# nightgoodl/ovmono3d

Measured on AMD Instinct MI355X. Metric: images/sec/GPU @512x512 DINOv2-L SFP; AP3D delta vs reference, higher is better.
Workload: dtype f16x3; 1 GPU; DINOv2 vitl14 + SFP + ROIHeads3DGDINO (native GroundingDINO Swin-B/BERT-base, 900 queries, 6 categories -> NMS) + ROIAlign + CubeHead + decode, batch 1/GPU, 512x512 synthetic -> network res 532 -> canvas 896 (T=4097), random-init weights (seed 0); precision=f16x3, parallelism=dp1 (image-sharded, no data-path collective)

## Files before the change

### ovmono3d_amd/csrc/gdino.hip

```cpp
#include <cmath>
#include <cstdio>
#include <cstdlib>
#include "det2d.hpp"
#include "dec_chain.hpp"
#include "gdino_model.hpp"

using namespace ovm;
using namespace ovm::gdino;

namespace ovm {
GdinoTune g_gdino_tune = {1, 1, 0, 1, 1, 1, 0};
void set_gdino_branches(int v) { g_gdino_tune.branches = v ? 1 : 0; }
void set_gdino_dec_chain(int v) { g_gdino_tune.dec_chain = v ? 1 : 0; }
void set_gdino_ffn_split(int v) { g_gdino_tune.ffn_split = v ? 1 : 0; }
void set_gdino_swin_fused(int v) { g_gdino_tune.swin_fused = v ? 1 : 0; }
void set_gdino_swin_tap(int v) { g_gdino_tune.swin_tap = v > 0 ? v : 0; }
void set_gdino_gemm256(int v) { g_gdino_tune.gemm256 = v ? 1 : 0; }
void set_gdino_mlp_fused(int v) { g_gdino_tune.mlp_fused = v < 0 ? 0 : (v > 2 ? 2 : v); }
}

namespace ovm {
namespace gdino {
namespace {

struct Feat { float* f; int h, w, C; };
struct DecScratch {
  float *tkv_all, *val_all;
  float *sine, *qh, *qpos, *qk, *vq, *ctx, *pre, *ow, *ffb, *b1, *b2, *delta;
  float* refs[2];
  bool chain; int ffn_chunks;
  float *ffn_x, *ffn_part;
};
struct State {
  float *tx, *text0, *text;
  std::vector<Feat> feats;
  float *vis0, *vis;
  float* ref; int* topk;
  float *hs, *last_ref, *hn;
  DecScratch d;
};

inline int now_cols(const OvmGdinoConfig& c) { return c.heads * c.n_levels * c.n_points * 3; }

void mha_core(Run& r, const float* q, int ldq, const float* k, int ldk, const float* v, int ldv, int Tq, int Tk, int heads, int D, const float* bias,
              int ldb, float* out, int ldo) {
  AttnF32Params a; memset(&a, 0, sizeof(a));
  const int dh = D / heads;
  a.q = q; a.k = k; a.v = v; a.ldq = ldq; a.ldk = ldk; a.ldv = ldv;
  a.sq2 = dh; a.sk2 = dh; a.sv2 = dh; a.o = out; a.ldo = ldo; a.so2 = dh;
  a.nb1 = 1; a.nb2 = heads; a.Tq = Tq; a.Tk = Tk; a.DH = dh; a.scale = 1.0f / sqrtf((float)dh);
  a.bias_b = bias; a.sbb = 0; a.ldbb = ldb;
// ... 129 lines not shown
    r.rowop(p);
    float* y = r.f32((size_t)h * w * C);
    GemmParams q = r.gp(pa, h * w, g->pe); q.C = y; q.ldc = C;
    r.gemm(q, EPI_STORE);
    r.ln(y, h * w, C, g->pe_ln, eps, nullptr, x);
    r.release(mk);
  }
  int ordinal = 0;
  for (size_t si = 0; si < g->stages.size(); ++si) {
    const SwinStage& stg = g->stages[si];
    const StageGeo& ge = pl->geo[si];
    const int ntok = h * w;
    for (size_t b = 0; b < stg.blocks.size(); ++b) swin_block(r, stg.blocks[b], ge.wm[b & 1], x, C, stg.nh, ntok, ++ordinal);
    if (stg.has_out) {
      float* f = r.f32((size_t)ntok * C);
      r.ln(x, ntok, C, stg.on, eps, nullptr, f);
      st.feats.push_back({f, h, w, C});
      r.tap("swin_stage" + std::to_string(st.feats.size()), f, (int64_t)ntok * C);
    }
    if (stg.has_red) { x = patch_merge(r, stg, ge, x, C); h = ge.h2; w = ge.w2; C = 2 * C; }
  }
}

void neck(Run& r, State& st) {
  OvmGdino* g = r.g; Plan* pl = r.pl;
  const OvmGdinoConfig& c = g->cfg;
  const int D = c.d_model, S = pl->S;
  st.vis0 = r.f32((size_t)S * D);
  st.vis = r.f32((size_t)S * D);
  const size_t mk = r.mark();
  for (int l = 0; l < c.n_levels; ++l) {
    const int n = pl->lh[l] * pl->lw[l];
    float* y = r.f32((size_t)n * D);
    const bool conv = l >= (int)st.feats.size();
    const Feat& f = conv ? st.feats.back() : st.feats[l];
    const int K = conv ? 9 * f.C : f.C;
    SplitBuf a = r.split((size_t)n, K);
    RowOpParams p = Run::rows(f.f, f.C, n, K); Run::into(p, a);
    if (conv) { p.idx = pl->conv_map; p.nidx = 9; p.seg = f.C; }
    r.rowop(p);
    GemmParams q = r.gp(a, n, g->inproj[l].w); q.C = y; q.ldc = D;
    r.gemm(q, EPI_STORE);
    if (r.go()) r.chk(ovm_g_groupnorm(y, 1, n, D, 32, g->inproj[l].gn.g, g->inproj[l].gn.b, 1e-5f, st.vis0 + (size_t)pl->lstart[l] * D, r.s_main), "groupnorm");
  }
  r.release(mk);
}

struct EncBufs {
  float* v; SplitBuf vsp; float *t, *qvv, *tkv; SplitBuf cv; float* ct;
  BiAttnWs bw; float *sc, *stat, *part, *bml;
  float *text2, *tqk, *tv, *tctx, *tff;
  SplitBuf vis_sp, visp_sp; float *val, *ow; SplitBuf dsp; float* pre; SplitBuf ff;
  bool ffn_fused;
};

void fusion_layer(Run& r, const EncLayer& ly, EncBufs& b, const float* vis_in, const float* text_in) {
  const OvmGdinoConfig& c = r.g->cfg;
  const int D = c.d_model, T = r.pl->T, S = r.pl->S, HF = c.heads / 2, E = c.ffn_dim / 2, dhf = E / HF;
  r.ln(vis_in, S, D, ly.lnv, c.eps, nullptr, b.v, &b.vsp);
  r.ln(text_in, T, D, ly.lnt, c.eps, nullptr, b.t);
  { GemmParams q = r.gp(b.vsp, S, ly.vqv); q.C = b.qvv; q.ldc = 2 * E; r.gemm(q, EPI_STORE); }
  r.lin(b.t, nullptr, D, T, ly.tkv, 0, nullptr, 0, b.tkv, 2 * E);
  if (!r.go()) return;
  BiAttnParams a; memset(&a, 0, sizeof(a));
  a.qv = b.qvv; a.ldq = 2 * E; a.kt = b.tkv; a.ldk = 2 * E; a.vv = b.qvv + E; a.ldvv = 2 * E; a.vt = b.tkv + E; a.ldvt = 2 * E;
  a.S = S; a.T = T; a.H = HF; a.dh = dhf; a.scale = 1.0f / sqrtf((float)dhf);
  a.cv_hi = b.cv.hi; a.cv_lo = b.cv.lo; a.ldcv = b.cv.ld; a.ct = b.ct; a.sc = b.sc; a.stat = b.stat; a.part = b.part; a.chunk = b.bw.chunk; a.nchunk = b.bw.nchunk;
// ... 5 lines not shown
  const OvmGdinoConfig& c = r.g->cfg;
  const int D = c.d_model, T = r.pl->T, E = c.ffn_dim / 2;
  r.fork(); r.on_text();
  r.lin(b.ct, nullptr, E, T, ly.ot, 0, b.t, D, b.text2, D);
  r.lin(b.text2, r.pl->text_pos, D, T, ly.te.qk, 0, nullptr, 0, b.tqk, 2 * D);
  r.lin(b.text2, nullptr, D, T, ly.te.v, 0, nullptr, 0, b.tv, D);
  mha_core(r, b.tqk, 2 * D, b.tqk + D, 2 * D, b.tv, D, T, T, ly.te.heads, D, r.pl->text_bias, T, b.tctx, D);
  r.lin(b.tctx, nullptr, D, T, ly.te.out, 0, b.text2, D, b.t, D);
  r.ln(b.t, T, D, ly.te_ln1, c.eps, nullptr, b.text2);
  r.lin(b.text2, nullptr, D, T, ly.te_fc1, 1, nullptr, 0, b.tff, ly.te_fc1.N);
  r.lin(b.tff, nullptr, ly.te_fc1.N, T, ly.te_fc2, 0, b.text2, D, b.t, D);
  r.ln(b.t, T, D, ly.te_ln2, c.eps, nullptr, text);
  r.on_image();
}

void deformable_layer(Run& r, const EncLayer& ly, EncBufs& b, float* vis) {
  const OvmGdinoConfig& c = r.g->cfg; Plan* pl = r.pl;
  const int D = c.d_model, S = pl->S, NOW = now_cols(c);
  { GemmParams q = r.gp(b.cv, S, ly.ov); q.C = vis; q.ldc = D; q.R = b.v; q.ldr = D; r.gemm(q, EPI_STORE); }
  {
    RowOpParams p = Run::rows(vis, D, S, D); Run::into(p, b.vis_sp);
    p.add = pl->pos; p.ld_add = D; p.add_rows = S; p.hi2 = b.visp_sp.hi; p.lo2 = b.visp_sp.lo; p.ldh2 = b.visp_sp.ld;
    r.rowop(p);
  }
  { GemmParams q = r.gp(b.vis_sp, S, ly.msda.value); q.C = b.val; q.ldc = D; r.gemm(q, EPI_STORE); }
  { GemmParams q = r.gp(b.visp_sp, S, ly.msda.offw); q.C = b.ow; q.ldc = NOW; r.gemm(q, EPI_STORE); }
  deform(r, b.val, D, b.ow, NOW, pl->ref, 2, 0, S, nullptr, &b.dsp);
  { GemmParams q = r.gp(b.dsp, S, ly.msda.out); q.C = b.pre; q.ldc = D; q.R = vis; q.ldr = D; r.gemm(q, EPI_STORE); }
  r.ln(b.pre, S, D, ly.de_ln1, c.eps, nullptr, b.v, &b.vsp);
  if (b.ffn_fused) {
    GemmParams q = r.gp(b.vsp, S, ly.de_fc2); q.C = b.pre; q.ldc = D; q.R = b.v; q.ldr = D;
    r.mlp_fused(b.vsp, S, ly.de_fc1, ly.de_fc2, 1, q, EPI_STORE);
  } else {
    { GemmParams q = r.gp(b.vsp, S, ly.de_fc1); q.Ohi = b.ff.hi; q.Olo = b.ff.lo; q.ldo = b.ff.ld; q.relu = 1; r.gemm(q, EPI_STORE); }
    { GemmParams q = r.gp(b.ff, S, ly.de_fc2); q.C = b.pre; q.ldc = D; q.R = b.v; q.ldr = D; r.gemm(q, EPI_STORE); }
  }
  r.ln(b.pre, S, D, ly.de_ln2, c.eps, nullptr, vis);
}

void encoder(Run& r, State& st) {
  const OvmGdinoConfig& c = r.g->cfg;
  const int D = c.d_model, T = r.pl->T, S = r.pl->S, HF = c.heads / 2, E = c.ffn_dim / 2, dhf = E / HF;
  r.join();
  const size_t mk = r.mark();
  EncBufs b;
  b.v = r.f32((size_t)S * D); b.vsp = r.split_for256((size_t)S, D);
  b.t = r.f32((size_t)T * D);
  b.qvv = r.f32((size_t)S * 2 * E);
  b.tkv = r.f32((size_t)T * 2 * E);
  b.cv = r.split((size_t)S, E);
  b.ct = r.f32((size_t)T * E);
  b.bw = biattn_workspace(S, T, HF, dhf, false);
  b.sc = b.bw.sc ? r.f32(b.bw.sc) : nullptr;
  b.stat = b.bw.stat ? r.f32(b.bw.stat) : nullptr;
  b.part = r.f32(b.bw.part);
  b.bml = b.bw.ml ? r.f32(2 * b.bw.ml) : nullptr;
  b.text2 = r.f32((size_t)T * D);
  b.tqk = r.f32((size_t)T * 2 * D); b.tv = r.f32((size_t)T * D); b.tctx = r.f32((size_t)T * D);
  b.tff = r.f32((size_t)T * c.ffn_dim);
  b.vis_sp = r.split((size_t)S, D); b.visp_sp = r.split((size_t)S, D);
  b.val = r.f32((size_t)S * D);
  b.ow = r.f32((size_t)S * now_cols(c));
  b.dsp = r.split((size_t)S, D);
  b.pre = r.f32((size_t)S * D);
  b.ffn_fused = b.vsp.il;
  for (auto& ly : r.g->enc) b.ffn_fused = b.ffn_fused && r.mlp_fused_ok(2, S, ly.de_fc1, ly.de_fc2, 1);
  if (!b.ffn_fused) b.ff = r.split((size_t)S, c.ffn_dim);
  const float* vis_in = st.vis0; const float* text_in = st.text0;
  for (auto& ly : r.g->enc) {
    fusion_layer(r, ly, b, vis_in, text_in);
    vis_in = st.vis; text_in = st.text;
    text_enhancer(r, ly, b, st.text);
    deformable_layer(r, ly, b, st.vis);
    r.join();
  }
  r.release(mk);
  r.tap("source_flatten", st.vis0, (int64_t)S * D);
  r.tap("enc_vision", st.vis, (int64_t)S * D);
  r.tap("enc_text", st.text, (int64_t)T * D);
}

void select_queries(Run& r, State& st) {
  OvmGdino* g = r.g; Plan* pl = r.pl;
  const OvmGdinoConfig& c = g->cfg;
  const int D = c.d_model, T = pl->T, S = pl->S, Q = c.num_queries;
  const hipStream_t s = r.s_main;
  float* ref = st.ref = r.f32((size_t)Q * 4);
  int* topk = st.topk = r.i32((size_t)Q);
// ... 26 lines not shown
  r.tap("topk", topk, Q);
  r.tap("init_ref", ref, (int64_t)Q * 4);
}

size_t decoder_inputs(Run& r, State& st) {
  OvmGdino* g = r.g; Plan* pl = r.pl;
  const OvmGdinoConfig& c = g->cfg;
  const int D = c.d_model, T = pl->T, S = pl->S, Q = c.num_queries, NL = (int)g->dec.size();
  DecScratch& d = st.d;
  st.hs = r.f32((size_t)Q * D);
  st.last_ref = r.f32((size_t)Q * 4);
  st.hn = r.f32((size_t)Q * D);
  const size_t mk = r.mark();
  d.tkv_all = r.f32((size_t)T * NL * 2 * D);
  r.lin(st.text, nullptr, D, T, g->dec_kv_text, 0, nullptr, 0, d.tkv_all, NL * 2 * D);
  SplitBuf vsp = r.split_for256((size_t)S, D);
  { RowOpParams p = Run::rows(st.vis, D, S, D); Run::into(p, vsp); r.rowop(p); }
  d.val_all = r.f32((size_t)S * NL * D);
  { GemmParams q = r.gp(vsp, S, g->dec_value); q.C = d.val_all; q.ldc = NL * D; r.gemm(q, EPI_STORE); }
  r.copy(st.hs, g->tgt, sizeof(float) * (size_t)Q * D, r.s_main);
  d.sine = r.f32((size_t)Q * 2 * D);
  d.qh = r.f32((size_t)Q * D); d.qpos = r.f32((size_t)Q * D);
  d.qk = r.f32((size_t)Q * 2 * D); d.vq = r.f32((size_t)Q * D); d.ctx = r.f32((size_t)Q * D);
  d.pre = r.f32((size_t)Q * D);
  d.ow = r.f32((size_t)Q * now_cols(c));
  d.ffb = r.f32((size_t)Q * c.ffn_dim);
  d.b1 = r.f32((size_t)Q * D); d.b2 = r.f32((size_t)Q * D); d.delta = r.f32((size_t)Q * 4);
  d.refs[0] = st.ref; d.refs[1] = r.f32((size_t)Q * 4);
  d.chain = pl->tune.dec_chain && dec_chain_supported(D, c.heads, c.ffn_dim, c.n_levels, c.n_points, T, g->precision);
  const int chunks = c.ffn_dim > 512 ? c.ffn_dim / 512 : 1;
  d.ffn_chunks = (d.chain && pl->tune.ffn_split && chunks > 1) ? chunks : 0;
  d.ffn_x = d.ffn_chunks ? r.f32((size_t)Q * D) : nullptr;
// ... 173 lines not shown
    (void)hipDeviceGetStreamPriorityRange(&lo, &hi);
    if (hipStreamCreateWithPriority(&g->aux, hipStreamNonBlocking, hi) != hipSuccess || hipEventCreateWithFlags(&g->ev_fork, hipEventDisableTiming) != hipSuccess ||
        hipEventCreateWithFlags(&g->ev_join, hipEventDisableTiming) != hipSuccess) {
      g->err = "could not create the text-branch stream"; return OVM_ERR_HIP;
    }
  }
  const OvmGdinoConfig& c = g->cfg;
  if (c.d_model % c.heads || c.n_levels > 8 || c.n_levels < 1 || c.swin_window <= 0) { g->err = "bad GroundingDINO config"; return OVM_ERR_INVALID; }
  OVM_HIP(g, hipSetDevice(device));
  const WeightMap wm(weights, n_weights);
  OVM_TRY(g, load_bert(g, wm));
  OVM_TRY(g, load_swin(g, wm));
  OVM_TRY(g, load_neck(g, wm));
  OVM_TRY(g, load_encoder(g, wm));
  OVM_TRY(g, load_decoder(g, wm));
  OVM_HIP(g, hipDeviceSynchronize());
  return OVM_OK;
}

int ovm_gdino_destroy(OvmGdino* g) {
  if (!g) return OVM_OK;
  (void)hipSetDevice(g->device);
  (void)hipDeviceSynchronize();
  for (Plan* p : g->plans) delete p;
  g->free_all();
  if (g->aux) (void)hipStreamDestroy(g->aux);
  if (g->ev_fork) (void)hipEventDestroy(g->ev_fork);
  if (g->ev_join) (void)hipEventDestroy(g->ev_join);
  delete g;
  return OVM_OK;
// ... 85 lines not shown
```

### ovmono3d_amd/csrc/gdino_load.hip

```cpp
#include <cmath>
#include "gdino_model.hpp"

namespace ovm {
namespace gdino {
namespace {

const std::string M = "model.";

int up_ln(OvmGdino* g, const WeightMap& wm, const std::string& prefix, Ln* ln) {
  OVM_TRY(g, upload_weight(g, wm, prefix + ".weight", -1, &ln->g));
  return upload_weight(g, wm, prefix + ".bias", -1, &ln->b);
}

int make_frag(OvmGdino* g, Lin* w) {
  std::vector<half_t> src; src.swap(w->img);
  if (g->precision != 3 || !w->hi) return OVM_OK;
  const int Npad = npad128(w->N), KS = w->Kpad / 32;
  const size_t n = (size_t)Npad * 2 * w->Kpad;
  if (src.size() != n) { g->err = "make_frag: the weight was packed without keeping its host image"; return OVM_ERR_INVALID; }
  std::vector<half_t> dst(n);
  for (int tile = 0; tile < Npad / 16; ++tile)
    for (int ks = 0; ks < KS; ++ks)
      for (int part = 0; part < 2; ++part)
        for (int lane = 0; lane < 64; ++lane) {
// ... 196 lines not shown
  {
    const int F = c.d_model / 2;
    std::vector<float> dt((size_t)F / 2);
    for (int i = 0; i < F / 2; ++i) dt[i] = powf(10000.0f, 2.f * (float)i / (float)F);
    OVM_TRY(g, upload_f32(g, dt.data(), dt.size(), &g->sine_dim_t));
  }
  for (int k = 0; k < 2; ++k) OVM_TRY(g, make_frag(g, &g->ref_head[k]));
  for (int i = 0; i < c.dec_layers; ++i) {
    DecLayer& ly = g->dec[i];
    for (Lin* w : {&ly.sa.qk, &ly.sa.v, &ly.sa.out, &ly.ca.q, &ly.ca.out, &ly.msda.offw, &ly.msda.out, &ly.fc1, &ly.fc2}) OVM_TRY(g, make_frag(g, w));
    if (i + 1 < c.dec_layers) for (int k = 0; k < 3; ++k) OVM_TRY(g, make_frag(g, &g->bbox[i][k]));
  }
  return OVM_OK;
}

}
}
```

### ovmono3d_amd/csrc/gdino_model.hpp

```cpp
#pragma once
#include <hip/hip_runtime.h>
#include <array>
#include <cstring>
#include <list>
#include <map>
#include <string>
#include <vector>
#include "../../include/ovm3d.h"
#include "gdino.hpp"
#include "kernels.hpp"
#include "loader.hpp"
#include "tower.hpp"

namespace ovm {

struct GdinoTune {
  int branches;
  int dec_chain;
  int ffn_split;
  int swin_fused;
  int gemm256;
  int mlp_fused;
  int swin_tap;
};
extern GdinoTune g_gdino_tune;

namespace gdino {

struct Lin : PackedLin {
  half_t* frag = nullptr;
  std::vector<half_t> img;
};
struct Ln { float* g = nullptr; float* b = nullptr; };
struct SplitBuf { half_t* hi = nullptr; half_t* lo = nullptr; int ld = 0; bool il = false; };

struct SwinBlock { Ln ln1, ln2; Lin qkv, proj, fc1, fc2; float* relbias = nullptr; };
struct SwinStage { std::vector<SwinBlock> blocks; int nh = 0, C = 0; bool has_red = false; Lin red; Ln dn; bool has_out = false; Ln on; };
struct BertLayer { Lin qkv, ao, fi, fo; Ln aln, oln; };
struct Mha { Lin qk, v, out; Lin q, kv; int heads = 0; };
struct MsdaW { Lin offw, value, out; };
struct EncLayer {
  Ln lnv, lnt; Lin vqv, tkv, ov, ot;
  Mha te; Ln te_ln1, te_ln2; Lin te_fc1, te_fc2;
  MsdaW msda; Ln de_ln1, de_ln2; Lin de_fc1, de_fc2;
};
struct DecLayer { Mha sa, ca; MsdaW msda; Ln ln1, ln2, ln3, ln4; Lin fc1, fc2; };

struct Plan;

struct Model : Loader {
  OvmGdinoConfig cfg;
  int device = 0;
  float* sine_dim_t = nullptr;
  float *word = nullptr, *posemb = nullptr, *typemb = nullptr; Ln emb_ln; int bertD = 0, n_pos = 0, vocab = 0;
  std::vector<BertLayer> bert;
// ... 19 lines not shown
};

}
}

struct OvmGdino : ovm::gdino::Model {};

namespace ovm {
namespace gdino {

int load_bert(OvmGdino* g, const WeightMap& wm);
int load_swin(OvmGdino* g, const WeightMap& wm);
int load_neck(OvmGdino* g, const WeightMap& wm);
int load_encoder(OvmGdino* g, const WeightMap& wm);
int load_decoder(OvmGdino* g, const WeightMap& wm);

struct WinMaps { int* win = nullptr; float* mask = nullptr; int nW = 0; };
struct StageGeo { int h = 0, w = 0; WinMaps wm[2]; int* merge = nullptr; int h2 = 0, w2 = 0; };

struct Plan {
  int H = 0, W = 0, T = 0;
  std::vector<int> ids, pids;
  GdinoTune tune = {};
  std::vector<void*> allocs; size_t bytes = 0;
  int* d_ids = nullptr; int* d_pids = nullptr; float* text_bias = nullptr; float* text_pos = nullptr;
  int Hp = 0, Wp = 0; int* pe_map = nullptr;
  std::vector<StageGeo> geo;
  int nlev = 0; int lh[8] = {0}, lw[8] = {0}, lstart[8] = {0}; int S = 0;
  int* conv_map = nullptr; int conv_h = 0, conv_w = 0;
  float* pos = nullptr; float* ref = nullptr; float* prop_logit = nullptr; int* valid_idx = nullptr;
  float* img = nullptr;
  char* arena = nullptr; size_t arena_cap = 0;
  float* gemm_ws = nullptr; size_t gemm_ws_cap = 0;
  unsigned long long* topk_keys = nullptr; int topk_N = 0;
  float* out_logits = nullptr; float* out_boxes = nullptr;
  std::map<std::string, std::pair<const void*, int64_t>> taps;
  hipGraph_t graph = nullptr; hipGraphExec_t exec = nullptr;
  long launches = 0;
  int mlp_fused_sites = 0;
  void drop_graph() {
    if (exec) { (void)hipGraphExecDestroy(exec); exec = nullptr; }
    if (graph) { (void)hipGraphDestroy(graph); graph = nullptr; }
  }
  ~Plan() {
    drop_graph();
// ... 132 lines not shown
```

### ovmono3d_amd/csrc/gdino_plan.hip

```cpp
#include <cmath>
#include <memory>
#include "gdino_model.hpp"

namespace ovm {
namespace gdino {
namespace {

template <typename T>
int pal(OvmGdino* g, Plan* pl, T** out, size_t count, const T* src = nullptr) {
  void* q = nullptr;
  size_t bytes = count * sizeof(T); if (bytes == 0) bytes = 16;
  OVM_HIP(g, hipMalloc(&q, bytes));
  pl->allocs.push_back(q); pl->bytes += bytes;
  if (src && count) OVM_HIP(g, hipMemcpy(q, src, count * sizeof(T), hipMemcpyHostToDevice));
  *out = (T*)q;
  return OVM_OK;
}
template <typename T>
int pup(OvmGdino* g, Plan* pl, const std::vector<T>& v, T** out) { return pal(g, pl, out, v.size(), v.data()); }

void text_masks(const std::vector<int>& ids, std::vector<char>* mask, std::vector<int>* pos) {
  const int T = (int)ids.size();
  mask->assign((size_t)T * T, 0);
  pos->assign(T, 0);
// ... 196 lines not shown
  }
  return OVM_OK;
}

int plan_scratch(OvmGdino* g, Plan* pl) {
  const OvmGdinoConfig& c = g->cfg;
  OVM_TRY(g, pal(g, pl, &pl->img, (size_t)pl->H * pl->W * 3));
  pl->topk_N = 2048; while (pl->topk_N < pl->S) pl->topk_N <<= 1;
  OVM_TRY(g, pal(g, pl, &pl->topk_keys, (size_t)pl->topk_N));
  OVM_TRY(g, pal(g, pl, &pl->out_logits, (size_t)c.num_queries * c.max_text_len));
  OVM_TRY(g, pal(g, pl, &pl->out_boxes, (size_t)c.num_queries * 4));
  pl->gemm_ws_cap = (size_t)64 << 20;
  return pal(g, pl, (char**)&pl->gemm_ws, pl->gemm_ws_cap);
}

}

int build_plan(OvmGdino* g, int H, int W, const std::vector<int>& ids, const std::vector<int>& pids, Plan** out) {
  std::unique_ptr<Plan> pl(new Plan());
  pl->H = H; pl->W = W; pl->T = (int)ids.size(); pl->ids = ids;
  pl->tune = g_gdino_tune; pl->tune.branches = g->branches;
  std::vector<std::pair<int, int>> feat_hw;
  OVM_TRY(g, plan_text(g, pl.get(), pids));
  OVM_TRY(g, plan_swin(g, pl.get(), &feat_hw));
  OVM_TRY(g, plan_levels(g, pl.get(), feat_hw));
  OVM_TRY(g, plan_encoder_tables(g, pl.get()));
  OVM_TRY(g, plan_scratch(g, pl.get()));
  *out = pl.release();
  return OVM_OK;
}

Plan* find_plan(OvmGdino* g, int H, int W, const std::vector<int>& ids, const std::vector<int>& pids) {
  for (auto it = g->plans.begin(); it != g->plans.end(); ++it) {
    Plan* p = *it;
    if (p->H == H && p->W == W && p->ids == ids && p->pids == pids) { g->plans.erase(it); return p; }
  }
  return nullptr;
}

void evict_plans(OvmGdino* g, const Plan* incoming) {
  const int maxp = g->cfg.max_plans > 0 ? g->cfg.max_plans : 128;
  const size_t budget = (size_t)(g->cfg.plan_budget_mb > 0 ? g->cfg.plan_budget_mb : 32768) << 20;
// ... 30 lines not shown
```

### ovmono3d_amd/csrc/gemm.hpp

```cpp
#pragma once
#include "common.hpp"

namespace ovm {

enum AMode { A_ROWMAJOR = 0, A_CONV3X3 = 1 };
enum Epi { EPI_STORE = 0, EPI_RESID = 1, EPI_GELU = 2, EPI_QKV = 3, EPI_PATCH = 4, EPI_CONVT = 5, EPI_SWIGLU = 6 };

struct GemmParams {
  const half_t* Ahi; const half_t* Alo; int lda;
  const half_t* Whi; const half_t* Wlo;
  int ldw;
  int a_il;
  int ksplit, kchunk; float* part;
  unsigned long long* stamps;
  float* part_ws; size_t part_cap;
  int ws_slot;
  int M, N, K;
  int cH, cW, cC;
  const float* bias;
  const float* gamma;
  float* X; int ldx;
  const int* row_map;
  float* C; int ldc;
  half_t* Ohi; half_t* Olo; int ldo;
  int o_il;
  int relu;
  const float* R; int ldr;
  const float* R2; int ldr2;
  int relu_o;
  int padH, padW;
  half_t *Qhi, *Qlo, *Khi, *Klo, *Vhi, *Vlo; int T, Tpad, heads; float qscale;
  const float* pos; int G2;
  int G, Cout;
  int main_tiles, tail_begin, M_total;
  int tail_waves;
};

template <int BK> __device__ __forceinline__ int swz_slot(int row, int chunk);
template <> __device__ __forceinline__ int swz_slot<64>(int row, int chunk) { return chunk ^ ((row >> 1) & 7); }
template <> __device__ __forceinline__ int swz_slot<32>(int row, int chunk) {
  return chunk ^ ((0x78 >> (2 * ((row >> 2) & 3))) & 3);
}
// ... 140 lines not shown
    const int q = n / p.Cout, co = n - q * p.Cout;
    const int a = q >> 1, bb = q & 1;
    const int j = m % p.G; const int t = m / p.G; const int i = t % p.G; const int b = t / p.G;
    const int ps = p.ldo > 0 ? p.ldo : p.Cout, bd = p.padH > 0 ? 1 : 0, side = 2 * p.G + 2 * bd;
    const size_t o = (((size_t)b * side + 2 * i + a + bd) * side + 2 * j + bb + bd) * ps + co;
    half4 h, l;
#pragma unroll
    for (int r = 0; r < 4; ++r) {
      const float bv = p.bias ? p.bias[co + r] : 0.f;
      half_t hh, ll; split_f16(v[r] + bv, hh, ll); h[r] = hh; l[r] = ll;
    }
    *(half4*)(p.Ohi + o) = h;
    if (p.Olo) *(half4*)(p.Olo + o) = l;
  } else {
    float o4[4];
#pragma unroll
    for (int r = 0; r < 4; ++r) {
      o4[r] = v[r] + b4[r];
      if (p.relu == 1) o4[r] = fmaxf(o4[r], 0.f); else if (p.relu == 2) o4[r] = gelu_erf(o4[r]);
      if (p.R && n + r < p.N) o4[r] += p.R[(size_t)m * p.ldr + n + r];
      if (p.R2 && n + r < p.N) o4[r] += p.R2[(size_t)m * p.ldr2 + n + r];
    }
    if (p.C) {
      float* c = p.C + (size_t)m * p.ldc + n;
      for (int r = 0; r < 4 && n + r < p.N; ++r) c[r] = o4[r];
    }
    if (p.Ohi) {
      size_t row = (size_t)m;
      if (p.padH > 0) {
        const int x = m % p.padW; const int t = m / p.padW; const int y = t % p.padH; const int b = t / p.padH;
        row = ((size_t)b * (p.padH + 2) + y + 1) * (p.padW + 2) + x + 1;
      }
      const size_t o = row * p.ldo + n;
      for (int r = 0; r < 4 && n + r < p.N; ++r) {
        half_t hh, ll; split_f16(p.relu_o ? fmaxf(o4[r], 0.f) : o4[r], hh, ll);
        p.Ohi[o + r] = hh;
        if (p.Olo) p.Olo[o + r] = ll;
      }
    }
  }
}

template <int NPASS, int EPI, int AMODE, bool AIL>
__device__ __forceinline__ void gemm_tail_body(const GemmParams& p, int tb);

template <int NPASS, int BK, int BM, int NSTAGE, int EPI, int AMODE, bool AIL = false>
__global__ __launch_bounds__(BM * 2) void gemm_kernel(const GemmParams p) {
  if ((int)blockIdx.x >= p.main_tiles) { gemm_tail_body<NPASS, EPI, AMODE, AIL>(p, (int)blockIdx.x - p.main_tiles); return; }
  extern __shared__ __attribute__((aligned(16))) char smem[];
  constexpr int NW = BM / 32;
  using SA = Side<NPASS, BK, AIL && NPASS == 3>;
  using SW = Side<NPASS, BK, NPASS == 3>;
// ... 444 lines not shown
```

### ovmono3d_amd/csrc/ops.hip

```cpp
#include <hip/hip_runtime.h>
#include <cstring>
#include <vector>
#include "../../include/ovm3d.h"
#include "kernels.hpp"
#include "det2d.hpp"
#include "gdino.hpp"
#include "tower.hpp"

using namespace ovm;

namespace {
__global__ void split_kernel(const float* __restrict__ x, int64_t n, half_t* __restrict__ hi, half_t* __restrict__ lo) {
  const int64_t i = (int64_t)blockIdx.x * blockDim.x + threadIdx.x;
  if (i >= n) return;
  half_t h, l; split_f16(x[i], h, l);
  hi[i] = h;
  if (lo) lo[i] = l;
}
__global__ void qkv_layout_kernel(const float* __restrict__ qkv, int B, int T, int Tpad, int heads,
                                  half_t* Qh, half_t* Ql, half_t* Kh, half_t* Kl, half_t* Vh, half_t* Vl) {
  const int D = heads * 64;
  const int64_t i = (int64_t)blockIdx.x * blockDim.x + threadIdx.x;
  const int64_t total = (int64_t)B * T * 3 * D;
  if (i >= total) return;
// ... 17 lines not shown
  y[i] = (float)hi[i] + (lo ? (float)lo[i] : 0.f);
}
struct Tmp {
  std::vector<void*> p;
  template <typename Tp> Tp* get(size_t n, bool zero = false) {
    void* q = nullptr;
    if (hipMalloc(&q, n * sizeof(Tp) + 16) != hipSuccess) return nullptr;
    if (zero) hipMemset(q, 0, n * sizeof(Tp) + 16);
    p.push_back(q);
    return (Tp*)q;
  }
  ~Tmp() { for (void* q : p) hipFree(q); }
};
}

namespace ovm { void set_use_gemm256(int v); void set_gdino_branches(int v); void msdeform_set_vec(int v); void set_gdino_dec_chain(int v); void set_gdino_gemm256(int v); void set_gdino_swin_fused(int v); void set_gdino_swin_tap(int v); void set_gdino_ffn_split(int v); void set_gdino_mlp_fused(int v); void gemm256_set_n192(int v); void set_gemm256_ksplit(int v); }

extern "C" {

int ovm_op_split_f16(const float* x, int64_t n, uint16_t* hi, uint16_t* lo, ovm_stream_t stream) {
  if (n <= 0) return OVM_OK;
  hipLaunchKernelGGL(split_kernel, dim3((unsigned)((n + 255) / 256)), dim3(256), 0, (hipStream_t)stream, x, n, (half_t*)hi, (half_t*)lo);
  return hipGetLastError() == hipSuccess ? OVM_OK : OVM_ERR_HIP;
}

static int g_op_gemm256 = 0;
static unsigned long long* g_gemm256_stamps = nullptr;

int ovm_op_gemm(const uint16_t* a_hi, const uint16_t* a_lo, int32_t lda, const uint16_t* w_hi, const uint16_t* w_lo,
                int32_t M, int32_t N, int32_t K, const float* bias, int32_t relu, float* c, int32_t ldc,
                int32_t precision, ovm_stream_t stream) {
// ... 313 lines not shown

int ovm_tune_set(const char* key, int32_t value) {
  if (!key) return OVM_ERR_INVALID;
  if (!strcmp(key, "gemm_bm")) { gemm_set_force_bm(value); return OVM_OK; }
  if (!strcmp(key, "gemm_stages")) { gemm_set_stages(value); return OVM_OK; }
  if (!strcmp(key, "gemm_splitk")) { gemm_set_splitk(value); return OVM_OK; }
  if (!strcmp(key, "gemm_tail")) { gemm_set_tail_rows(value); return OVM_OK; }
  if (!strcmp(key, "attn_waves")) { attn_set_waves(value); return OVM_OK; }
  if (!strcmp(key, "attn_pp")) {
#ifndef OVM_DIAG
    if (value < 0 || value > 1) return OVM_ERR_INVALID;
#endif
    attn_set_pp(value); return OVM_OK;
  }
  if (!strcmp(key, "gdino_mlp_fused")) { ovm::set_gdino_mlp_fused(value); return OVM_OK; }
  if (!strcmp(key, "gdino_ffn_split")) { ovm::set_gdino_ffn_split(value); return OVM_OK; }
  if (!strcmp(key, "gdino_swin_tap")) { ovm::set_gdino_swin_tap(value); return OVM_OK; }
  if (!strcmp(key, "gdino_swin_fused")) { ovm::set_gdino_swin_fused(value); return OVM_OK; }
  if (!strcmp(key, "gdino_gemm256")) { ovm::set_gdino_gemm256(value); return OVM_OK; }
  if (!strcmp(key, "gdino_dec_chain")) { ovm::set_gdino_dec_chain(value); return OVM_OK; }
  if (!strcmp(key, "msdeform_vec")) { msdeform_set_vec(value); return OVM_OK; }
  if (!strcmp(key, "attn_q64")) { attn_set_q64(value); return OVM_OK; }
  if (!strcmp(key, "attn_prio")) { attn_set_prio(value); return OVM_OK; }
  if (!strcmp(key, "attn_lds_pad")) { attn_set_lds_pad(value); return OVM_OK; }
  if (!strcmp(key, "attn_tail")) { attn_set_tail_rows(value); return OVM_OK; }
  if (!strcmp(key, "attn_tail_split")) { attn_set_tail_split(value); return OVM_OK; }
  if (!strcmp(key, "glin_small_max_tiles")) { glinear_set_small_max_tiles(value); return OVM_OK; }
  if (!strcmp(key, "glin_target_blocks")) { gemm_small_set(value, -1); return OVM_OK; }
  if (!strcmp(key, "gbmm_tiled")) { gbmm_set_tiled(value); return OVM_OK; }
  if (!strcmp(key, "glin_stages")) { gemm_small_set_stages(value); return OVM_OK; }
// ... 92 lines not shown
```

Before: 52.37 images/sec.

## Fold positional offsets into plan tables and merge encoder value/offset GEMMs

Adds an opt-in encoder mode that precomputes pos·W_offsets per layer at plan time, so one concatenated GEMM yields both value and sampling offsets plus attention weights. This removes the separate pos-add rowop, the second split buffer and one GEMM per layer. A second opt-in mode makes swin feature outputs and the last encoder layernorm emit f16 hi/lo splits directly, so the neck and decoder skip re-splitting. The GEMM epilogue also gains vectorized f32x4 and half4 stores and an offset residual (r_n0). Both encoder modes default to off, so by default only the vectorized epilogue and the extra weight packing at load time take effect.

```diff
diff --git a/ovmono3d_amd/csrc/gdino.hip b/ovmono3d_amd/csrc/gdino.hip
--- a/ovmono3d_amd/csrc/gdino.hip
+++ b/ovmono3d_amd/csrc/gdino.hip
@@ -9,7 +9,7 @@
 using namespace ovm::gdino;
 
 namespace ovm {
-GdinoTune g_gdino_tune = {1, 1, 0, 1, 1, 1, 0};
+GdinoTune g_gdino_tune = {1, 1, 0, 1, 1, 1, 0, 0, 0};
 void set_gdino_branches(int v) { g_gdino_tune.branches = v ? 1 : 0; }
 void set_gdino_dec_chain(int v) { g_gdino_tune.dec_chain = v ? 1 : 0; }
 void set_gdino_ffn_split(int v) { g_gdino_tune.ffn_split = v ? 1 : 0; }
@@ -17,13 +17,15 @@
 void set_gdino_swin_tap(int v) { g_gdino_tune.swin_tap = v > 0 ? v : 0; }
 void set_gdino_gemm256(int v) { g_gdino_tune.gemm256 = v ? 1 : 0; }
 void set_gdino_mlp_fused(int v) { g_gdino_tune.mlp_fused = v < 0 ? 0 : (v > 2 ? 2 : v); }
+void set_gdino_enc_fold(int v) { g_gdino_tune.enc_fold = (v < 0 || v > 3) ? 0 : v; }
+void set_gdino_enc_tap(int v) { g_gdino_tune.enc_tap = v ? 1 : 0; }
 }
 
 namespace ovm {
 namespace gdino {
 namespace {
 
-struct Feat { float* f; int h, w, C; };
+struct Feat { float* f; int h, w, C; SplitBuf sp; };
 struct DecScratch {
   float *tkv_all, *val_all;
   float *sine, *qh, *qpos, *qk, *vq, *ctx, *pre, *ow, *ffb, *b1, *b2, *delta;
@@ -35,6 +37,7 @@
   float *tx, *text0, *text;
   std::vector<Feat> feats;
   float *vis0, *vis;
+  SplitBuf dec_vsp;
   float* ref; int* topk;
   float *hs, *last_ref, *hn;
   DecScratch d;
@@ -194,8 +197,10 @@
     for (size_t b = 0; b < stg.blocks.size(); ++b) swin_block(r, stg.blocks[b], ge.wm[b & 1], x, C, stg.nh, ntok, ++ordinal);
     if (stg.has_out) {
       float* f = r.f32((size_t)ntok * C);
-      r.ln(x, ntok, C, stg.on, eps, nullptr, f);
-      st.feats.push_back({f, h, w, C});
+      SplitBuf sp;
+      if (pl->tune.prod_split() && (int)st.feats.size() < g->cfg.n_levels) sp = r.split((size_t)ntok, C);
+      r.ln(x, ntok, C, stg.on, eps, nullptr, f, sp.hi ? &sp : nullptr);
+      st.feats.push_back({f, h, w, C, sp});
       r.tap("swin_stage" + std::to_string(st.feats.size()), f, (int64_t)ntok * C);
     }
     if (stg.has_red) { x = patch_merge(r, stg, ge, x, C); h = ge.h2; w = ge.w2; C = 2 * C; }
@@ -215,10 +220,13 @@
     const bool conv = l >= (int)st.feats.size();
     const Feat& f = conv ? st.feats.back() : st.feats[l];
     const int K = conv ? 9 * f.C : f.C;
-    SplitBuf a = r.split((size_t)n, K);
-    RowOpParams p = Run::rows(f.f, f.C, n, K); Run::into(p, a);
-    if (conv) { p.idx = pl->conv_map; p.nidx = 9; p.seg = f.C; }
-    r.rowop(p);
+    SplitBuf a = f.sp;
+    if (conv || !a.hi) {
+      a = r.split((size_t)n, K);
+      RowOpParams p = Run::rows(f.f, f.C, n, K); Run::into(p, a);
+      if (conv) { p.idx = pl->conv_map; p.nidx = 9; p.seg = f.C; }
+      r.rowop(p);
+    }
     GemmParams q = r.gp(a, n, g->inproj[l].w); q.C = y; q.ldc = D;
     r.gemm(q, EPI_STORE);
     if (r.go()) r.chk(ovm_g_groupnorm(y, 1, n, D, 32, g->inproj[l].gn.g, g->inproj[l].gn.b, 1e-5f, st.vis0 + (size_t)pl->lstart[l] * D, r.s_main), "groupnorm");
@@ -231,6 +239,8 @@
   BiAttnWs bw; float *sc, *stat, *part, *bml;
   float *text2, *tqk, *tv, *tctx, *tff;
   SplitBuf vis_sp, visp_sp; float *val, *ow; SplitBuf dsp; float* pre; SplitBuf ff;
+  float* voff;
+  float *tap_vis = nullptr, *tap_voff = nullptr; half_t *tap_hi = nullptr, *tap_lo = nullptr;
   bool ffn_fused;
 };
 
@@ -266,18 +276,38 @@
   r.on_image();
 }
 
-void deformable_layer(Run& r, const EncLayer& ly, EncBufs& b, float* vis) {
+void deformable_layer(Run& r, const EncLayer& ly, EncBufs& b, float* vis, int li, const SplitBuf* out_sp) {
   const OvmGdinoConfig& c = r.g->cfg; Plan* pl = r.pl;
   const int D = c.d_model, S = pl->S, NOW = now_cols(c);
-  { GemmParams q = r.gp(b.cv, S, ly.ov); q.C = vis; q.ldc = D; q.R = b.v; q.ldr = D; r.gemm(q, EPI_STORE); }
-  {
-    RowOpParams p = Run::rows(vis, D, S, D); Run::into(p, b.vis_sp);
-    p.add = pl->pos; p.ld_add = D; p.add_rows = S; p.hi2 = b.visp_sp.hi; p.lo2 = b.visp_sp.lo; p.ldh2 = b.visp_sp.ld;
-    r.rowop(p);
-  }
-  { GemmParams q = r.gp(b.vis_sp, S, ly.msda.value); q.C = b.val; q.ldc = D; r.gemm(q, EPI_STORE); }
-  { GemmParams q = r.gp(b.visp_sp, S, ly.msda.offw); q.C = b.ow; q.ldc = NOW; r.gemm(q, EPI_STORE); }
-  deform(r, b.val, D, b.ow, NOW, pl->ref, 2, 0, S, nullptr, &b.dsp);
+  if (pl->tune.fold()) {
+    { GemmParams q = r.gp(b.cv, S, ly.ov); q.C = vis; q.ldc = D; q.R = b.v; q.ldr = D; q.Ohi = b.vis_sp.hi; q.Olo = b.vis_sp.lo; q.ldo = b.vis_sp.ld; r.gemm(q, EPI_STORE); }
+    { GemmParams q = r.gp(b.vis_sp, S, ly.msda.voff); q.C = b.voff; q.ldc = D + NOW; q.R = pl->enc_P[li]; q.ldr = NOW; q.r_n0 = D; r.gemm(q, EPI_STORE); }
+    deform(r, b.voff, D + NOW, b.voff + D, D + NOW, pl->ref, 2, 0, S, nullptr, &b.dsp);
+  } else {
+    { GemmParams q = r.gp(b.cv, S, ly.ov); q.C = vis; q.ldc = D; q.R = b.v; q.ldr = D; r.gemm(q, EPI_STORE); }
+    {
+      RowOpParams p = Run::rows(vis, D, S, D); Run::into(p, b.vis_sp);
+      p.add = pl->pos; p.ld_add = D; p.add_rows = S; p.hi2 = b.visp_sp.hi; p.lo2 = b.visp_sp.lo; p.ldh2 = b.visp_sp.ld;
+      r.rowop(p);
+    }
+    { GemmParams q = r.gp(b.vis_sp, S, ly.msda.value); q.C = b.val; q.ldc = D; r.gemm(q, EPI_STORE); }
+    { GemmParams q = r.gp(b.visp_sp, S, ly.msda.offw); q.C = b.ow; q.ldc = NOW; r.gemm(q, EPI_STORE); }
+    deform(r, b.val, D, b.ow, NOW, pl->ref, 2, 0, S, nullptr, &b.dsp);
+  }
+  if (li == 0 && b.tap_vis) {
+    const size_t nsp = (size_t)S * b.vis_sp.ld * sizeof(half_t);
+    r.tap("enc_pos", pl->pos, (int64_t)S * D);
+    r.copy(b.tap_vis, vis, sizeof(float) * (size_t)S * D, r.s_main); r.tap("enc_vis0", b.tap_vis, (int64_t)S * D);
+    r.copy(b.tap_hi, b.vis_sp.hi, nsp, r.s_main); r.tap("enc_vis0_hi", b.tap_hi, (int64_t)(nsp / 4));
+    if (b.vis_sp.lo) { r.copy(b.tap_lo, b.vis_sp.lo, nsp, r.s_main); r.tap("enc_vis0_lo", b.tap_lo, (int64_t)(nsp / 4)); }
+    if (pl->tune.fold()) {
+      r.copy(b.tap_voff, b.voff, sizeof(float) * (size_t)S * (D + NOW), r.s_main); r.tap("enc_voff0", b.tap_voff, (int64_t)S * (D + NOW));
+      r.tap("enc_P0", pl->enc_P[0], (int64_t)S * NOW);
+    } else {
+      r.copy(b.tap_voff, b.val, sizeof(float) * (size_t)S * D, r.s_main); r.tap("enc_val0", b.tap_voff, (int64_t)S * D);
+      r.copy(b.tap_voff + (size_t)S * D, b.ow, sizeof(float) * (size_t)S * NOW, r.s_main); r.tap("enc_ow0", b.tap_voff + (size_t)S * D, (int64_t)S * NOW);
+    }
+  }
   { GemmParams q = r.gp(b.dsp, S, ly.msda.out); q.C = b.pre; q.ldc = D; q.R = vis; q.ldr = D; r.gemm(q, EPI_STORE); }
   r.ln(b.pre, S, D, ly.de_ln1, c.eps, nullptr, b.v, &b.vsp);
   if (b.ffn_fused) {
@@ -287,15 +317,22 @@
     { GemmParams q = r.gp(b.vsp, S, ly.de_fc1); q.Ohi = b.ff.hi; q.Olo = b.ff.lo; q.ldo = b.ff.ld; q.relu = 1; r.gemm(q, EPI_STORE); }
     { GemmParams q = r.gp(b.ff, S, ly.de_fc2); q.C = b.pre; q.ldc = D; q.R = b.v; q.ldr = D; r.gemm(q, EPI_STORE); }
   }
-  r.ln(b.pre, S, D, ly.de_ln2, c.eps, nullptr, vis);
+  r.ln(b.pre, S, D, ly.de_ln2, c.eps, nullptr, vis, out_sp);
 }
 
 void encoder(Run& r, State& st) {
   const OvmGdinoConfig& c = r.g->cfg;
   const int D = c.d_model, T = r.pl->T, S = r.pl->S, HF = c.heads / 2, E = c.ffn_dim / 2, dhf = E / HF;
+  const int NOW = now_cols(c), NE = (int)r.g->enc.size();
   r.join();
+  EncBufs b;
+  if (r.pl->tune.prod_split() && NE > 0) st.dec_vsp = r.split_for256((size_t)S, D);
+  if (r.pl->tune.enc_tap && NE > 0) {
+    const size_t nsp = (size_t)S * ((D + 63) / 64 * 64) * sizeof(half_t);
+    b.tap_vis = r.f32((size_t)S * D); b.tap_voff = r.f32((size_t)S * (D + NOW));
+    b.tap_hi = (half_t*)r.alloc(nsp); b.tap_lo = (half_t*)r.alloc(nsp);
+  }
   const size_t mk = r.mark();
-  EncBufs b;
   b.v = r.f32((size_t)S * D); b.vsp = r.split_for256((size_t)S, D);
   b.t = r.f32((size_t)T * D);
   b.qvv = r.f32((size_t)S * 2 * E);
@@ -310,20 +347,28 @@
   b.text2 = r.f32((size_t)T * D);
   b.tqk = r.f32((size_t)T * 2 * D); b.tv = r.f32((size_t)T * D); b.tctx = r.f32((size_t)T * D);
   b.tff = r.f32((size_t)T * c.ffn_dim);
-  b.vis_sp = r.split((size_t)S, D); b.visp_sp = r.split((size_t)S, D);
-  b.val = r.f32((size_t)S * D);
-  b.ow = r.f32((size_t)S * now_cols(c));
+  b.vis_sp = r.split((size_t)S, D);
+  b.val = b.ow = b.voff = nullptr;
+  if (r.pl->tune.fold()) {
+    if ((int)r.pl->enc_P.size() != NE || D % 4) { r.fail(OVM_ERR_INVALID, "encoder: the plan has no offsets tables"); return; }
+    b.voff = r.f32((size_t)S * (D + NOW));
+  } else {
+    b.visp_sp = r.split((size_t)S, D);
+    b.val = r.f32((size_t)S * D);
+    b.ow = r.f32((size_t)S * NOW);
+  }
   b.dsp = r.split((size_t)S, D);
   b.pre = r.f32((size_t)S * D);
   b.ffn_fused = b.vsp.il;
   for (auto& ly : r.g->enc) b.ffn_fused = b.ffn_fused && r.mlp_fused_ok(2, S, ly.de_fc1, ly.de_fc2, 1);
   if (!b.ffn_fused) b.ff = r.split((size_t)S, c.ffn_dim);
   const float* vis_in = st.vis0; const float* text_in = st.text0;
-  for (auto& ly : r.g->enc) {
+  for (int li = 0; li < NE; ++li) {
+    const EncLayer& ly = r.g->enc[li];
     fusion_layer(r, ly, b, vis_in, text_in);
     vis_in = st.vis; text_in = st.text;
     text_enhancer(r, ly, b, st.text);
-    deformable_layer(r, ly, b, st.vis);
+    deformable_layer(r, ly, b, st.vis, li, (li == NE - 1 && st.dec_vsp.hi) ? &st.dec_vsp : nullptr);
     r.join();
   }
   r.release(mk);
@@ -380,8 +425,11 @@
   const size_t mk = r.mark();
   d.tkv_all = r.f32((size_t)T * NL * 2 * D);
   r.lin(st.text, nullptr, D, T, g->dec_kv_text, 0, nullptr, 0, d.tkv_all, NL * 2 * D);
-  SplitBuf vsp = r.split_for256((size_t)S, D);
-  { RowOpParams p = Run::rows(st.vis, D, S, D); Run::into(p, vsp); r.rowop(p); }
+  SplitBuf vsp = st.dec_vsp;
+  if (!vsp.hi) {
+    vsp = r.split_for256((size_t)S, D);
+    RowOpParams p = Run::rows(st.vis, D, S, D); Run::into(p, vsp); r.rowop(p);
+  }
   d.val_all = r.f32((size_t)S * NL * D);
   { GemmParams q = r.gp(vsp, S, g->dec_value); q.C = d.val_all; q.ldc = NL * D; r.gemm(q, EPI_STORE); }
   r.copy(st.hs, g->tgt, sizeof(float) * (size_t)Q * D, r.s_main);
@@ -585,6 +633,7 @@
   OVM_TRY(g, load_neck(g, wm));
   OVM_TRY(g, load_encoder(g, wm));
   OVM_TRY(g, load_decoder(g, wm));
+  OVM_TRY(g, load_encoder_merged(g, wm));
   OVM_HIP(g, hipDeviceSynchronize());
   return OVM_OK;
 }
diff --git a/ovmono3d_amd/csrc/gdino_load.hip b/ovmono3d_amd/csrc/gdino_load.hip
--- a/ovmono3d_amd/csrc/gdino_load.hip
+++ b/ovmono3d_amd/csrc/gdino_load.hip
@@ -234,5 +234,19 @@
   return OVM_OK;
 }
 
-}
-}
+int load_encoder_merged(OvmGdino* g, const WeightMap& wm) {
+  for (size_t i = 0; i < g->enc.size(); ++i) {
+    MsdaW& m = g->enc[i].msda;
+    const std::string p = M + "encoder.layers." + std::to_string(i) + ".deformable_layer.self_attn.";
+    OVM_TRY(g, pack_cat(g, wm, {p + "value_proj", p + "sampling_offsets", p + "attention_weights"}, &m.voff, false));
+    if (m.voff.N != m.value.N + m.offw.N || m.voff.Kpad != m.value.Kpad) { g->err = "merged value | offsets weight shape"; return OVM_ERR_SHAPE; }
+    const float* bv; OVM_TRY(g, find_weight(g, wm, p + "value_proj.bias", m.value.N, &bv));
+    std::vector<float> b((size_t)m.voff.N, 0.f);
+    for (int n = 0; n < m.value.N; ++n) b[n] = bv[n];
+    OVM_TRY(g, upload_f32(g, b.data(), b.size(), &m.voff.bias));
+  }
+  return OVM_OK;
+}
+
+}
+}
diff --git a/ovmono3d_amd/csrc/gdino_model.hpp b/ovmono3d_amd/csrc/gdino_model.hpp
--- a/ovmono3d_amd/csrc/gdino_model.hpp
+++ b/ovmono3d_amd/csrc/gdino_model.hpp
@@ -22,6 +22,10 @@
   int gemm256;
   int mlp_fused;
   int swin_tap;
+  int enc_fold;
+  int enc_tap;
+  bool fold() const { return enc_fold == 1 || enc_fold == 2; }
+  bool prod_split() const { return enc_fold == 1 || enc_fold == 3; }
 };
 extern GdinoTune g_gdino_tune;
 
@@ -38,7 +42,7 @@
 struct SwinStage { std::vector<SwinBlock> blocks; int nh = 0, C = 0; bool has_red = false; Lin red; Ln dn; bool has_out = false; Ln on; };
 struct BertLayer { Lin qkv, ao, fi, fo; Ln aln, oln; };
 struct Mha { Lin qk, v, out; Lin q, kv; int heads = 0; };
-struct MsdaW { Lin offw, value, out; };
+struct MsdaW { Lin offw, value, out; Lin voff; };
 struct EncLayer {
   Ln lnv, lnt; Lin vqv, tkv, ov, ot;
   Mha te; Ln te_ln1, te_ln2; Lin te_fc1, te_fc2;
@@ -88,6 +92,7 @@
 int load_neck(OvmGdino* g, const WeightMap& wm);
 int load_encoder(OvmGdino* g, const WeightMap& wm);
 int load_decoder(OvmGdino* g, const WeightMap& wm);
+int load_encoder_merged(OvmGdino* g, const WeightMap& wm);
 
 struct WinMaps { int* win = nullptr; float* mask = nullptr; int nW = 0; };
 struct StageGeo { int h = 0, w = 0; WinMaps wm[2]; int* merge = nullptr; int h2 = 0, w2 = 0; };
@@ -103,6 +108,7 @@
   int nlev = 0; int lh[8] = {0}, lw[8] = {0}, lstart[8] = {0}; int S = 0;
   int* conv_map = nullptr; int conv_h = 0, conv_w = 0;
   float* pos = nullptr; float* ref = nullptr; float* prop_logit = nullptr; int* valid_idx = nullptr;
+  std::vector<float*> enc_P;
   float* img = nullptr;
   char* arena = nullptr; size_t arena_cap = 0;
   float* gemm_ws = nullptr; size_t gemm_ws_cap = 0;
diff --git a/ovmono3d_amd/csrc/gdino_plan.hip b/ovmono3d_amd/csrc/gdino_plan.hip
--- a/ovmono3d_amd/csrc/gdino_plan.hip
+++ b/ovmono3d_amd/csrc/gdino_plan.hip
@@ -234,6 +234,22 @@
   return pal(g, pl, (char**)&pl->gemm_ws, pl->gemm_ws_cap);
 }
 
+int plan_offset_tables(OvmGdino* g, Plan* pl) {
+  const OvmGdinoConfig& c = g->cfg;
+  const int S = pl->S, D = c.d_model, NOW = c.heads * c.n_levels * c.n_points * 3;
+  if (!gemm_small_supported(pl->pos, D, D)) { g->err = "offsets tables: d_model must be a multiple of 4"; return OVM_ERR_SHAPE; }
+  pl->enc_P.assign(g->enc.size(), nullptr);
+  for (size_t i = 0; i < g->enc.size(); ++i) {
+    const Lin& w = g->enc[i].msda.offw;
+    if (w.N != NOW || w.K != D) { g->err = "offsets tables: sampling-offsets weight shape"; return OVM_ERR_SHAPE; }
+    OVM_TRY(g, pal(g, pl, &pl->enc_P[i], (size_t)S * NOW));
+    OVM_TRY(g, launch_gemm_small_ex(pl->pos, nullptr, D, S, D, w.hi, w.lo, NOW, w.Kpad, w.bias, 0, nullptr, 0, pl->enc_P[i], NOW, g->precision,
+                                    pl->gemm_ws, pl->gemm_ws_cap, nullptr));
+  }
+  OVM_HIP(g, hipDeviceSynchronize());
+  return OVM_OK;
+}
+
 }
 
 int build_plan(OvmGdino* g, int H, int W, const std::vector<int>& ids, const std::vector<int>& pids, Plan** out) {
@@ -246,6 +262,7 @@
   OVM_TRY(g, plan_levels(g, pl.get(), feat_hw));
   OVM_TRY(g, plan_encoder_tables(g, pl.get()));
   OVM_TRY(g, plan_scratch(g, pl.get()));
+  if (pl->tune.fold()) OVM_TRY(g, plan_offset_tables(g, pl.get()));
   *out = pl.release();
   return OVM_OK;
 }
diff --git a/ovmono3d_amd/csrc/gemm.hpp b/ovmono3d_amd/csrc/gemm.hpp
--- a/ovmono3d_amd/csrc/gemm.hpp
+++ b/ovmono3d_amd/csrc/gemm.hpp
@@ -26,6 +26,7 @@
   int o_il;
   int relu;
   const float* R; int ldr;
+  int r_n0;
   const float* R2; int ldr2;
   int relu_o;
   int padH, padW;
@@ -196,16 +197,28 @@
     if (p.Olo) *(half4*)(p.Olo + o) = l;
   } else {
     float o4[4];
+    float r4[4] = {0.f, 0.f, 0.f, 0.f};
+    if (p.R) {
+      if (full && n >= p.r_n0 && !((p.ldr | p.r_n0) & 3) && !((uintptr_t)p.R & 15)) {
+        const f32x4 t = *(const f32x4*)(p.R + (size_t)m * p.ldr + n - p.r_n0);
+        r4[0] = t[0]; r4[1] = t[1]; r4[2] = t[2]; r4[3] = t[3];
+      } else {
+#pragma unroll
+        for (int r = 0; r < 4; ++r)
+          if (n + r < p.N && n + r >= p.r_n0) r4[r] = p.R[(size_t)m * p.ldr + n + r - p.r_n0];
+      }
+    }
 #pragma unroll
     for (int r = 0; r < 4; ++r) {
       o4[r] = v[r] + b4[r];
       if (p.relu == 1) o4[r] = fmaxf(o4[r], 0.f); else if (p.relu == 2) o4[r] = gelu_erf(o4[r]);
-      if (p.R && n + r < p.N) o4[r] += p.R[(size_t)m * p.ldr + n + r];
+      if (p.R && n + r < p.N && n + r >= p.r_n0) o4[r] += r4[r];
       if (p.R2 && n + r < p.N) o4[r] += p.R2[(size_t)m * p.ldr2 + n + r];
     }
     if (p.C) {
       float* c = p.C + (size_t)m * p.ldc + n;
-      for (int r = 0; r < 4 && n + r < p.N; ++r) c[r] = o4[r];
+      if (full && !(p.ldc & 3) && !((uintptr_t)p.C & 15)) *(f32x4*)c = (f32x4){o4[0], o4[1], o4[2], o4[3]};
+      else for (int r = 0; r < 4 && n + r < p.N; ++r) c[r] = o4[r];
     }
     if (p.Ohi) {
       size_t row = (size_t)m;
@@ -214,10 +227,18 @@
         row = ((size_t)b * (p.padH + 2) + y + 1) * (p.padW + 2) + x + 1;
       }
       const size_t o = row * p.ldo + n;
-      for (int r = 0; r < 4 && n + r < p.N; ++r) {
-        half_t hh, ll; split_f16(p.relu_o ? fmaxf(o4[r], 0.f) : o4[r], hh, ll);
-        p.Ohi[o + r] = hh;
-        if (p.Olo) p.Olo[o + r] = ll;
+      if (full && !(p.ldo & 3) && !(((uintptr_t)p.Ohi | (uintptr_t)p.Olo) & 7)) {
+        half4 h, l;
+#pragma unroll
+        for (int r = 0; r < 4; ++r) { half_t hh, ll; split_f16(p.relu_o ? fmaxf(o4[r], 0.f) : o4[r], hh, ll); h[r] = hh; l[r] = ll; }
+        *(half4*)(p.Ohi + o) = h;
+        if (p.Olo) *(half4*)(p.Olo + o) = l;
+      } else {
+        for (int r = 0; r < 4 && n + r < p.N; ++r) {
+          half_t hh, ll; split_f16(p.relu_o ? fmaxf(o4[r], 0.f) : o4[r], hh, ll);
+          p.Ohi[o + r] = hh;
+          if (p.Olo) p.Olo[o + r] = ll;
+        }
       }
     }
   }
diff --git a/ovmono3d_amd/csrc/ops.hip b/ovmono3d_amd/csrc/ops.hip
--- a/ovmono3d_amd/csrc/ops.hip
+++ b/ovmono3d_amd/csrc/ops.hip
@@ -55,7 +55,7 @@
 };
 }
 
-namespace ovm { void set_use_gemm256(int v); void set_gdino_branches(int v); void msdeform_set_vec(int v); void set_gdino_dec_chain(int v); void set_gdino_gemm256(int v); void set_gdino_swin_fused(int v); void set_gdino_swin_tap(int v); void set_gdino_ffn_split(int v); void set_gdino_mlp_fused(int v); void gemm256_set_n192(int v); void set_gemm256_ksplit(int v); }
+namespace ovm { void set_use_gemm256(int v); void set_gdino_branches(int v); void msdeform_set_vec(int v); void set_gdino_dec_chain(int v); void set_gdino_gemm256(int v); void set_gdino_swin_fused(int v); void set_gdino_swin_tap(int v); void set_gdino_ffn_split(int v); void set_gdino_mlp_fused(int v); void set_gdino_enc_fold(int v); void set_gdino_enc_tap(int v); void gemm256_set_n192(int v); void set_gemm256_ksplit(int v); }
 
 extern "C" {
 
@@ -399,6 +399,8 @@
     attn_set_pp(value); return OVM_OK;
   }
   if (!strcmp(key, "gdino_mlp_fused")) { ovm::set_gdino_mlp_fused(value); return OVM_OK; }
+  if (!strcmp(key, "gdino_enc_fold")) { ovm::set_gdino_enc_fold(value); return OVM_OK; }
+  if (!strcmp(key, "gdino_enc_tap")) { ovm::set_gdino_enc_tap(value); return OVM_OK; }
   if (!strcmp(key, "gdino_ffn_split")) { ovm::set_gdino_ffn_split(value); return OVM_OK; }
   if (!strcmp(key, "gdino_swin_tap")) { ovm::set_gdino_swin_tap(value); return OVM_OK; }
   if (!strcmp(key, "gdino_swin_fused")) { ovm::set_gdino_swin_fused(value); return OVM_OK; }
```

Measured after the change: 53.65 images/sec, median of 6. 2.4% higher.
